# jhidalgocarrio/slam-localization

Hardware: AMD Instinct MI355X
Metric: filter predict+update steps/sec (higher is better)
Workload: dtype f64

## Files before the change

### slam-localization_amd/csrc/slk_step_fast.hpp

```cpp
#pragma once
#ifdef SLK_STAMPS
#define SLK_FSTAMP(i) do { SLK_STAMP_NR(i); if (a.stop > 0 && a.stop == (i)) return true; } while (0)
#define SLK_WSTAMP(w, i) do { if (tid == 64 * (w) && a.dbg) a.dbg[(size_t)bidx * 32 + (i)] = clock64(); } while (0)
#define SLK_FBAIL(code) do { SLK_NOTE(28, code); return false; } while (0)
#else
#define SLK_FSTAMP(i) do { } while (0)
#define SLK_WSTAMP(w, i) do { } while (0)
#define SLK_FBAIL(code) return false
#endif

namespace slk {

template <int K> struct FastShape {
    static constexpr int N = 12 + 6 * K, Nq = 13 + 7 * K, S = 2 * N + 1, NSO3 = K + 1;
    static constexpr int NT = (N + 15) / 16, NTL = NT * (NT + 1) / 2, NKS = (N + 3) / 4;
    static constexpr int NROT = 3 * NSO3;
    static constexpr int NP = 3 * K * K + 15 * K + 6;
    static constexpr int NIT = NP + NSO3;
    static constexpr int RND = (NIT + 255) / 256;
    static constexpr int oLt = 0;
    static constexpr int oMu = oLt + NTL * 256;
    static constexpr int oRef = oMu + ((Nq + 7) & ~7);
    static constexpr int oDelta = oRef + ((Nq + 7) & ~7);
    static constexpr int oMd = oDelta + 64;
    static constexpr int oD0 = oMd + 32;
    static constexpr int oD0s = oD0 + 32;
    static constexpr int oPd = oD0s + 32;
    static constexpr int oCq = oPd + 64;
    static constexpr int oStr = oCq + 40;
    static constexpr int oInts = oStr + 64;
    static constexpr int oTab = oInts + 32;
    static constexpr int oMsq = oTab + 28;
    static constexpr int oU = oTab + 32;
    static constexpr int uYp = 0, uW = 0, uDZ = 1088, uSm = 1600, uMdiag = 1664, uB = 1728, uInnov = 1792, uDz0 = 1800, uTmp = 1808;
    static constexpr int USZ = (NKS * 128 > 1936) ? NKS * 128 : 1936;
    static constexpr int total = oU + USZ;
};

static_assert(FastShape<8>::total * 8 * 4 <= 160 * 1024 && FastShape<7>::total * 8 * 4 <= 160 * 1024, "four workgroups per CU");

__host__ __device__ inline int fast_step_lds_doubles(int k)
{
    switch (k) {
    case 4: return FastShape<4>::total;
    case 5: return FastShape<5>::total;
    case 6: return FastShape<6>::total;
    case 7: return FastShape<7>::total;
    case 8: return FastShape<8>::total;
    default: return 0;
    }
}

__device__ __forceinline__ double wave_sum_f64(double x) { return readlane_f64(wave_inclusive_scan(x), 63); }

template <int N> __device__ __forceinline__ int fast_rho(int t)
{
    if (t >= N) return 31;
    if (t < 12) return (t >= 3 && t < 6) ? t - 3 : 31;
    const int cc = (t - 12) / 6, r = (t - 12) - 6 * cc;
    return r >= 3 ? 3 * cc + r : 31;
}
__device__ __forceinline__ int fast_vec_storage(int t)
{
    if (t < 12) return t < 3 ? t : (t < 6 ? -1 : t + 1);
    const int cc = (t - 12) / 6, r = (t - 12) - 6 * cc;
    return r < 3 ? 13 + 7 * cc + r : -1;
}

__device__ const double fast_series_table[26] = {
    0x1.1d8d32755f8fbp-29, 0x1.27e40964b47d4p-22, 0x1.a01a00fb1bc6fp-16, 0x1.6c16c16bdd04ep-10, 0x1.5555555555421p-5, 0x1.fffffffffffffp-2,
    0x1.ac53ce336f805p-26, 0x1.71dd113fb7905p-19, 0x1.a01a01061c190p-13, 0x1.11111110ecfb3p-7, 0x1.555555555548fp-3,
    0x1.78be0a9b1dd1fp-5, 0x1.0b3340fe2ed9ap-4, 0x1.3ab708d770276p-4, 0x1.7459b99bfc19bp-4, 0x1.c71c5f4b9c2adp-4, 0x1.24924907fa636p-3, 0x1.999999996d307p-3, 0x1.5555555555481p-2,
    0.0, 0.0, 0.0, 0.0, 0.0, 0.0, 0.0};

__device__ __forceinline__ bool wave_all(bool p) { return __builtin_amdgcn_ballot_w64(!p) == 0ull; }

template <int NV, bool WIDE>
__device__ __forceinline__ void so3_exp_tab_path(const double *T, const double (&v)[NV][3], const double (&x)[NV], Quat (&q)[NV])
{
    double y[NV], cc[NV], ss[NV];
#pragma unroll
    for (int i = 0; i < NV; ++i) y[i] = WIDE ? -0.0625 * x[i] : -x[i];
    {
        const double c0 = T[0], s0 = T[6];
#pragma unroll
        for (int i = 0; i < NV; ++i) { cc[i] = c0; ss[i] = s0; }
    }
#pragma unroll
    for (int k = 1; k < 5; ++k) {
        const double ck = T[k], sk = T[6 + k];
#pragma unroll
        for (int i = 0; i < NV; ++i) { cc[i] = fma(cc[i], y[i], ck); ss[i] = fma(ss[i], y[i], sk); }
    }
    {
        const double c5 = T[5];
#pragma unroll
        for (int i = 0; i < NV; ++i) {
            cc[i] = fma(cc[i], y[i], c5);
            cc[i] = fma(cc[i], y[i], 1.0);
            ss[i] = fma(ss[i], y[i], 1.0);
        }
    }
#pragma unroll
    for (int i = 0; i < NV; ++i) {
        double m = 0.5 * ss[i], w = cc[i];
        if (WIDE) {
            m *= 0.25;
#pragma unroll
            for (int rep = 0; rep < 2; ++rep) {
                const double w2 = fma(2.0 * w, w, -1.0);
                m = 2.0 * w * m;
                w = w2;
            }
        }
        q[i] = Quat{m * v[i][0], m * v[i][1], m * v[i][2], w};
    }
}
template <int NV, bool FLAG>
__device__ __forceinline__ bool so3_exp_tab_impl(const double *T, const double (&v)[NV][3], Quat (&q)[NV], int *flag)
{
    double x[NV];
    unsigned hm = 0;
#pragma unroll
    for (int i = 0; i < NV; ++i) {
        x[i] = 0.25 * (v[i][0] * v[i][0] + v[i][1] * v[i][1] + v[i][2] * v[i][2]);
        const unsigned hi = (unsigned)__double2hiint(x[i]);
        hm = hi > hm ? hi : hm;
    }
    if (wave_all(nonneg_hi_below(hm, HI_QUARTER))) {
        so3_exp_tab_path<NV, false>(T, v, x, q);
        return true;
    }
    so3_exp_tab_path<NV, true>(T, v, x, q);
    const bool ok = nonneg_hi_below(hm, HI_FOUR);
    if (!FLAG) return ok;
    if (!wave_all(ok)) *flag = 1;
    return true;
}
__device__ __forceinline__ Quat qmul_exp(const Quat &a, const Quat &b)
{
    Quat o;
    o.w = fma(-a.z, b.z, fma(-a.y, b.y, fma(a.w, b.w, -(a.x * b.x))));
    o.x = fma(-a.z, b.y, fma(a.y, b.z, fma(a.x, b.w, a.w * b.x)));
    o.y = fma(-a.x, b.z, fma(a.z, b.x, fma(a.y, b.w, a.w * b.y)));
    o.z = fma(-a.y, b.x, fma(a.x, b.y, fma(a.z, b.w, a.w * b.z)));
    return o;
}
template <int NV>
__device__ __forceinline__ bool so3_exp_tab(const double *T, const double (&v)[NV][3], Quat (&q)[NV])
{
    return so3_exp_tab_impl<NV, false>(T, v, q, nullptr);
}
template <int NV>
__device__ __forceinline__ void so3_exp_tab_flag(const double *T, const double (&v)[NV][3], Quat (&q)[NV], int *flag)
{
    so3_exp_tab_impl<NV, true>(T, v, q, flag);
}
template <int NV>
__device__ __forceinline__ bool so3_log_tab(const double *T, const Quat (&q)[NV], double (&d)[NV][3])
{
    double y[NV], sc[NV], f[NV];
    bool small = true;
#pragma unroll
    for (int i = 0; i < NV; ++i) {
        const double n2 = q[i].x * q[i].x + q[i].y * q[i].y + q[i].z * q[i].z, ws = q[i].w * fabs(q[i].w);
        small = small && (n2 * 16.0 < ws);
        y[i] = n2;
    }
    const bool wide = !wave_all(small);
    if (!wide) {
#pragma unroll
        for (int i = 0; i < NV; ++i) {
            const double r = rcp_refined(q[i].w);
            sc[i] = 2.0 * r;
            y[i] = -(y[i] * r * r);
        }
    } else {
#pragma unroll
        for (int i = 0; i < NV; ++i) {
            const double n2 = y[i], aw = fabs(q[i].w);
            const double r = rcp_refined(1.0 + aw);
            double k = r, t2 = n2 * r * r;
#pragma unroll
            for (int rep = 0; rep < 2; ++rep) {
                const double a1 = 1.0 + t2;
                double sq, rs;
                rsqrt_pivot(a1, sq, rs);
                const double den = fma(a1, rs, 1.0);
                const double rd = rcp_refined(den);
                k *= rd;
                t2 *= rd * rd;
            }
            sc[i] = (q[i].w < 0.0) ? -16.0 * k : 16.0 * k;
            y[i] = -t2;
        }
    }
    {
        const double a0 = T[11];
#pragma unroll
        for (int i = 0; i < NV; ++i) f[i] = a0;
    }
#pragma unroll
    for (int k = 1; k < 8; ++k) {
        const double ak = T[11 + k];
#pragma unroll
        for (int i = 0; i < NV; ++i) f[i] = fma(f[i], y[i], ak);
    }
#pragma unroll
    for (int i = 0; i < NV; ++i) {
        f[i] = fma(f[i], y[i], 1.0);
        const double sv = sc[i] * f[i];
        d[i][0] = sv * q[i].x; d[i][1] = sv * q[i].y; d[i][2] = sv * q[i].z;
    }
    return true;
}

template <int E0, int CNT>
__device__ __forceinline__ void fast_scan_entries(const double (&av)[8], double (&G)[20])
{
#pragma unroll
    for (int e = 0; e < CNT; ++e) {
        constexpr int dummy = 0; (void)dummy;
        const int q = E0 + e;
        const int r = (q >= 1) + (q >= 3) + (q >= 6) + (q >= 10) + (q >= 15) + (q >= 21) + (q >= 28), cc = q - r * (r + 1) / 2;
        const double pr = av[r] * av[cc];
        G[e] = wave_inclusive_scan(pr) - pr;
    }
}

template <int K> struct FastPairTable {
    unsigned long long v[FastShape<K>::NP];
    constexpr FastPairTable() : v{}
    {
        int p = 0;
        for (int b = 0; b <= K; ++b) {
            const int to = b ? 9 + 6 * b : 3;
            for (int j = 0; j < to + 3; ++j, ++p) {
                unsigned long long a[3] = {0, 0, 0};
                for (int cc = 0; cc < 3; ++cc) {
                    const int t = to + cc, I = t >> 4, Jc = j >> 4;
                    a[cc] = (unsigned long long)(FastShape<K>::oLt + (Jc <= I ? (I * (I + 1) / 2 + Jc) * 256 + (j & 15) * 16 + (t & 15) : 16));
                }
                const int rho = 3 * b;
                const unsigned long long e0 = (unsigned long long)(((j >> 2) * 2 + (rho >> 4)) * 64 + (j & 3) * 16 + (rho & 15));
                const unsigned long long sd = (b == 1 && j >= 16) ? (unsigned long long)(j - 15) : 0ull;
                v[p] = a[0] | (a[1] << 13) | ((unsigned long long)b << 26) | (sd << 30) | (a[2] << 32) | (e0 << 45);
            }
        }
    }
};
template <int K> struct FastPairTableHolder { static __device__ const FastPairTable<K> tab; };
template <int K> __device__ const FastPairTable<K> FastPairTableHolder<K>::tab = FastPairTable<K>();

#define SLK_G(r, c) Gf[(r) * ((r) + 1) / 2 + (c)]
__device__ __forceinline__ bool fast_ldm_columns(double (&Gf)[36], const double *dZi, const double *Sm, unsigned kept, int lane, int N,
                                                 double *Wb, double *mdiag)
{
    const bool live = lane < N;
    const bool full = kept == 0xffu;
    double y[8];
    bool ok = true;
#pragma unroll
    for (int j = 0; j < 8; ++j) {
        if (full) {
#pragma unroll
            for (int r = j; r < 8; ++r) SLK_G(r, j) = Sm[r + 8 * j] - SLK_G(r, j);
        } else {
            const bool kj = (kept >> j) & 1u;
#pragma unroll
            for (int r = j; r < 8; ++r) {
                const bool in = kj && ((kept >> r) & 1u);
                const double sv = Sm[in ? r + 8 * j : 0];
                SLK_G(r, j) = in ? sv - SLK_G(r, j) : ((r == j) ? 1.0 : 0.0);
            }
        }
        double d = SLK_G(j, j);
#pragma unroll
        for (int p = 0; p < j; ++p) d = fma(-SLK_G(j, p), SLK_G(j, p), d);
        ok = ok && (d > 0.0);
        double sq, rs;
        rsqrt_pivot(d, sq, rs);
        SLK_G(j, j) = rs;
#pragma unroll
        for (int i = j + 1; i < 8; ++i) {
            double v = SLK_G(i, j);
#pragma unroll
            for (int p = 0; p < j; ++p) v = fma(-SLK_G(i, p), SLK_G(j, p), v);
            SLK_G(i, j) = v * rs;
        }
        const double aj = dZi[(j >> 1) * 128 + 2 * lane + (j & 1)];
        double sacc = ((kept >> j) & 1u) ? 0.5 * aj : 0.0;
#pragma unroll
        for (int p = 0; p < j; ++p) sacc = fma(-SLK_G(j, p), y[p], sacc);
        y[j] = sacc * rs;
    }
    double dj = 1.0;
#pragma unroll
    for (int c = 0; c < 8; ++c) dj = fma(-y[c], y[c], dj);
    ok = ok && (dj > 0.0);
    double sqd, rsd;
    rsqrt_pivot(dj, sqd, rsd);
    const double sc = -0.5 * rsd;
#pragma unroll
    for (int c = 7; c >= 0; --c) {
        double sacc = y[c];
#pragma unroll
        for (int p = c + 1; p < 8; ++p) sacc = fma(-SLK_G(p, c), y[p], sacc);
        y[c] = sacc * SLK_G(c, c);
        Wb[bw_idx(lane, c)] = live ? y[c] * sc : 0.0;
    }
    mdiag[lane] = live ? sqd : 1.0;
    return __all(ok) != 0;
}
#undef SLK_G

template <int NT, class FillFn>
__device__ __forceinline__ void ldm_product_tiled(double *Lt, const double *dZi, const double *Wb, const double *mdiag, int lane,
                                                  int wave, int JB, FillFn fill)
{
    const int c = lane & 15, g = lane >> 4;
    const int lw = (g >> 1) * 128 + 2 * c + (g & 1);
    constexpr int MAXT = (NT == 4) ? 4 : 2;
    d4 acc[MAXT];
#pragma unroll
    for (int q = 0; q < MAXT; ++q) acc[q] = d4{0.0, 0.0, 0.0, 0.0};
#pragma unroll
    for (int I = 0; I < NT; ++I)
#pragma unroll
        for (int J = 0; J <= I; ++J) {
            if (ldm_tile_wave<NT>(I, J) != wave || J > JB) continue;
            d4 a = {0.0, 0.0, 0.0, 0.0};
            const double wf0 = Wb[32 * J + lw], wf1 = Wb[256 + 32 * J + lw];
#pragma unroll
            for (int Kb = J; Kb <= I; ++Kb) {
                if (Kb > JB) continue;
                d4 mt = {0.0, 0.0, 0.0, 0.0};
                const double a0 = dZi[32 * Kb + lw], a1 = dZi[256 + 32 * Kb + lw];
                double lf[4];
#pragma unroll
                for (int s = 0; s < 4; ++s) lf[s] = Lt[(I * (I + 1) / 2 + Kb) * 256 + 64 * s + lane];
                mt = __builtin_amdgcn_mfma_f64_16x16x4f64(a0, wf0, mt, 0, 0, 0);
                mt = __builtin_amdgcn_mfma_f64_16x16x4f64(a1, wf1, mt, 0, 0, 0);
                if (Kb == J) {
                    const double dg = mdiag[16 * J + c];
#pragma unroll
                    for (int r = 0; r < 4; ++r) {
                        const int row = g + 4 * r;
                        mt[r] = (row > c) ? mt[r] : ((row == c) ? dg : 0.0);
                    }
                }
#pragma unroll
                for (int s = 0; s < 4; ++s) a = __builtin_amdgcn_mfma_f64_16x16x4f64(mt[s], lf[s], a, 0, 0, 0);
            }
            acc[ldm_tile_slot<NT>(I, J)] = a;
        }
    __syncthreads();
#pragma unroll
    for (int I = 0; I < NT; ++I)
#pragma unroll
        for (int J = 0; J <= I; ++J) {
            if (ldm_tile_wave<NT>(I, J) != wave || J > JB) continue;
            const d4 a = acc[ldm_tile_slot<NT>(I, J)];
#pragma unroll
            for (int r = 0; r < 4; ++r) Lt[(I * (I + 1) / 2 + J) * 256 + 64 * r + lane] = a[r];
        }
    fill();
    __syncthreads();
}

template <int K> struct FastEE {
    using F = FastShape<K>;
    static constexpr int EES = 40;
    static constexpr int NTE = F::NROT > 16 ? 2 : 1;
    static constexpr int PAD = 16 * NTE - 1;
    static constexpr int BLO = F::NSO3 - 1 < 5 ? F::NSO3 - 1 : 5;
    static constexpr int CLO = (BLO ? 9 + 6 * BLO : 3) + 3;
    static constexpr int KS0 = ((CLO + 3) / 4 < F::NKS) ? (CLO + 3) / 4 : F::NKS;
    static constexpr int KS1 = F::NKS;
    __host__ __device__ static constexpr int wave_of(int hi, int hj) { return hi == 0 ? 0 : (hj == 0 ? 2 : 3); }
};
static_assert(32 * FastEE<8>::EES <= FastShape<4>::USZ, "EE fits the union region");

template <int K, int HI, int HJ>
__device__ __forceinline__ d4 fast_ee_tile(const double *Et, int lane)
{
    constexpr int KE = HJ == 0 ? FastEE<K>::KS0 : FastEE<K>::KS1;
    d4 acc = {0.0, 0.0, 0.0, 0.0};
#pragma unroll
    for (int ks = 0; ks < KE; ++ks) {
        const double fj = Et[ks * 128 + HJ * 64 + lane];
        const double fi = HI == HJ ? fj : Et[ks * 128 + HI * 64 + lane];
        acc = __builtin_amdgcn_mfma_f64_16x16x4f64(fi, fj, acc, 0, 0, 0);
    }
    return acc;
}
template <int K, int HI, int HJ>
__device__ __forceinline__ void fast_ee_publish(double *ee, int lane, const d4 &acc)
{
    constexpr int EES = FastEE<K>::EES;
    const int c = lane & 15, g = lane >> 4;
#pragma unroll
    for (int r = 0; r < 4; ++r) {
        ee[(16 * HI + g + 4 * r) * EES + 16 * HJ + c] = acc[r];
        if (HI != HJ) ee[(16 * HJ + c) * EES + 16 * HI + g + 4 * r] = acc[r];
    }
}

template <int K> __host__ __device__ constexpr unsigned fast_rho_pack(int I, int G)
{
    constexpr int N = FastShape<K>::N, PAD = FastEE<K>::PAD;
    unsigned w = 0;
    for (int r = 0; r < 4; ++r) {
        const int t = 16 * I + G + 4 * r;
        int rho = PAD;
        if (t < N) {
            if (t < 12) rho = (t >= 3 && t < 6) ? t - 3 : PAD;
            else { const int cc = (t - 12) / 6, q = (t - 12) - 6 * cc; rho = q >= 3 ? 3 * cc + q : PAD; }
        }
        w |= (unsigned)rho << (8 * r);
    }
    return w;
}

template <int K, int J>
__device__ __forceinline__ void fast_rebuild_col(const double *Lt, const double *str, int lane, d4 (&acc)[FastShape<K>::NT])
{
    using F = FastShape<K>;
    constexpr int NT = F::NT;
    constexpr int KEND = (4 * J + 4 + (J == 0 ? 1 : 0) < F::NKS) ? 4 * J + 4 + (J == 0 ? 1 : 0) : F::NKS;
#pragma unroll
    for (int ks = 0; ks < KEND; ++ks) {
        double fo[NT];
#pragma unroll
        for (int I = J; I < NT; ++I) {
            const int Kc = ks >> 2;
            fo[I] = (Kc <= I) ? Lt[(I * (I + 1) / 2 + Kc) * 256 + (ks & 3) * 64 + lane] : str[lane];
        }
#pragma unroll
        for (int I = J; I < NT; ++I) acc[I - J] = __builtin_amdgcn_mfma_f64_16x16x4f64(fo[I], fo[J], acc[I - J], 0, 0, 0);
    }
}

template <int K, int J>
__device__ __forceinline__ void fast_store_col(const double *pd, const double *ee, double *bufs, double *oP, int lane,
                                               d4 (&acc)[FastShape<K>::NT], bool lower_only)
{
    using F = FastShape<K>;
    constexpr int NT = F::NT, N = F::N, EES = FastEE<K>::EES, PAD = FastEE<K>::PAD;
    const int c = lane & 15, g = lane >> 4;
    {
        const int rj = fast_rho<N>(16 * J + c);
        const double bf = pd[g == 0 ? 32 + rj : (g == 1 ? rj : 31)];
#pragma unroll
        for (int I = J; I < NT; ++I) {
            const int ri = fast_rho<N>(16 * I + c);
            const double af = pd[g == 0 ? ri : (g == 1 ? 32 + ri : 31)];
            acc[I - J] = __builtin_amdgcn_mfma_f64_16x16x4f64(af, bf, acc[I - J], 0, 0, 0);
        }
        const double *eec = ee + (rj & PAD);
#pragma unroll
        for (int I = J; I < NT; ++I) {
            const unsigned rw = g == 0 ? fast_rho_pack<K>(I, 0) : (g == 1 ? fast_rho_pack<K>(I, 1) : (g == 2 ? fast_rho_pack<K>(I, 2) : fast_rho_pack<K>(I, 3)));
#pragma unroll
            for (int r = 0; r < 4; ++r) acc[I - J][r] += eec[((rw >> (8 * r)) & 0xffu) * EES];
        }
    }
    double *o = oP + c + g * N;
#pragma unroll
    for (int I = J; I < NT; ++I) {
#pragma unroll
        for (int r = 0; r < 4; ++r) {
            const bool full = 16 * I + 4 * r + 3 < N && 16 * J + 15 < N;
            if (I > J && lower_only) continue;
            if (16 * I + 4 * r < N && (full || (16 * I + 4 * r + g < N && 16 * J + c < N)))
                o[16 * J + (16 * I + 4 * r) * N] = acc[I - J][r];
        }
        if (I > J) {
            double *buf = bufs + (I * (I - 1) / 2 + J) * 272;
#pragma unroll
            for (int r = 0; r < 4; ++r) buf[c * 17 + g + 4 * r] = acc[I - J][r];
            wave_sync();
#pragma unroll
            for (int q = 0; q < 4; ++q) {
                const double v = buf[(g + 4 * q) * 17 + c];
                const bool full = 16 * I + 15 < N;
                if (full || 16 * I + c < N) o[16 * I + (16 * J + 4 * q) * N] = v;
            }
        }
    }
}

template <int K>
__device__ __forceinline__ bool msckf_step_fast(const KArgs &a, double *smem)
{
    using F = FastShape<K>;
    constexpr int N = F::N, Nq = F::Nq, S = F::S, NSO3 = F::NSO3, NT = F::NT, NKS = F::NKS, NROT = F::NROT;
    constexpr int NP = F::NP;
    constexpr int NTHREADS = 256;
    if (a.mm != SLK_MM_FEATURE_PROJ || a.gate == 2 || a.emit != 0 || a.rebuild_prec != 0 || !a.mp || a.m != 8) return false;
    const int bidx = blockIdx.x, tid = threadIdx.x, lane = tid & 63;
    const int wave = __builtin_amdgcn_readfirstlane(tid >> 6);
    const int c16 = lane & 15, g4 = lane >> 4;
    double *Lt = smem + F::oLt, *mu = smem + F::oMu, *ref = smem + F::oRef, *delta = smem + F::oDelta, *md32 = smem + F::oMd;
    double *d0 = smem + F::oD0, *d0s = smem + F::oD0s, *pd = smem + F::oPd, *cq = smem + F::oCq, *str = smem + F::oStr, *U = smem + F::oU;
    int *ints = reinterpret_cast<int *>(smem + F::oInts);
    double *T = smem + F::oTab, *msq = smem + F::oMsq;
    double *Yp = U + F::uYp, *Wb = U + F::uW, *dZi = U + F::uDZ, *Sm = U + F::uSm, *mdiag = U + F::uMdiag, *bvec = U + F::uB;
    double *innov = U + F::uInnov, *dz0 = U + F::uDz0, *tmpS = U + F::uTmp, *Et = U;
    const double *gmean = a.mean + (size_t)bidx * Nq;
    const double *gP = a.P + (size_t)bidx * N * N;
    const double *mp = a.mp + (size_t)bidx * a.mp_stride;
    SLK_STAMP_NR(0);

    int jmax = 0, bad;
    const bool here = a.wsfail == nullptr;
    {
        const double *gL = here ? gP : a.wsL + (size_t)bidx * pk_size(N);
        const int t = lane, It = t >> 4;
        const int lbase = (It * (It + 1) / 2) * 256 + wave * 16 + (t & 15);
        double v[16];
        if (!here) {
#pragma unroll
            for (int u = 0; u < 16; ++u) {
                const int j = 4 * u + wave;
                const bool in = j < N && t >= j && t < N;
                v[u] = gL[in ? pkcol(N, j) + t : 0];
            }
        }
        const double mu0 = (tid < Nq) ? gmean[tid] : 0.0;
        const int t0 = (tid && tid < NSO3) ? 9 + 6 * tid : 3;
        const double pdg = gP[t0 * (N + 1)] + gP[(t0 + 1) * (N + 1)] + gP[(t0 + 2) * (N + 1)];
        const double tabv = fast_series_table[tid < 26 ? tid : 25];
        bad = here ? 0 : (a.wsfail[bidx] >= 0);
        bool ok = true;
#pragma unroll
        for (int f = 0; f < 4; ++f) {
            const double cf = mp[4 * f + 3];
            ok = ok && (cf >= 0.0) && (cf <= (double)K);
            const int cp = ok ? (int)cf : 0, tp = cp ? 6 + 6 * cp : 0;
            jmax = (tp + 5 > jmax) ? tp + 5 : jmax;
        }
        bad |= !ok;
        if (tid < NSO3) bad |= !(pdg < 9.869604401089358);
        if (tid < Nq) mu[tid] = mu0;
        if (tid < 64) { str[tid] = 0.0; pd[tid] = 0.0; ints[tid] = 0; }
        if (tid < 32) { d0[tid] = 0.0; md32[tid] = 0.0; }
        if (tid < 26) T[tid] = tabv;
        if (!here) {
#pragma unroll
            for (int u = 0; u < 16; ++u) {
                const int j = 4 * u + wave;
                const bool in = j < N && t >= j && t < N;
                if ((u >> 2) < NT && It >= (u >> 2) && It < NT) Lt[lbase + (u >> 2) * 256 + (u & 3) * 64] = in ? v[u] : 0.0;
            }
        }
        if (here) {
            d4 fa[CholM<NT>::NTL];
            if (wave == 0) cholm_load_t_exact<NT, N>(fa, gP, lane);
            else {
                double2 *Lt2 = reinterpret_cast<double2 *>(Lt);
                for (int e = tid - 64; e < CholM<NT>::NTL * 128; e += NTHREADS - 64) Lt2[e] = double2{0.0, 0.0};
            }
            __syncthreads();
            if (wave == 0) bad |= cholp_factor<NT, 2, N>(fa, Lt, N, U, lane) >= 0;
        }
    }
    if (__syncthreads_or(bad)) SLK_FBAIL(2);
    SLK_FSTAMP(3);

    {
        const int f = wave;
        const int cp = (int)mp[4 * f + 3];
        const int tp = cp ? 6 + 6 * cp : 0, sp = cp ? 6 + 7 * cp : 0;
        const double fx = mp[4 * f], fy = mp[4 * f + 1], fz = mp[4 * f + 2];
        const int j = lane, Jc = j >> 4;
        const bool act = j < tp + 6;
        double l[6], x[7];
#pragma unroll
        for (int q = 0; q < 6; ++q) {
            const int t = tp + q, I = t >> 4;
            const bool in = act && Jc <= I;
            l[q] = Lt[in ? (I * (I + 1) / 2 + Jc) * 256 + (j & 15) * 16 + (t & 15) : 16];
        }
#pragma unroll
        for (int q = 0; q < 7; ++q) x[q] = mu[sp + q];
        double zp0, zp1, zm0, zm1;
        {
            const double rv[2][3] = {{l[3], l[4], l[5]}, {-l[3], -l[4], -l[5]}};
            Quat ex[2];
            so3_exp_tab_flag<2>(T, rv, ex, ints + 50);
            const Quat qx = Quat{x[3], x[4], x[5], x[6]};
            double lx, ly, lz;
            auto quot = [](double lx_, double ly_, double lz_, double &q0, double &q1) __attribute__((always_inline)) {
                const double r = rcp_refined(lz_);
                q0 = lx_ * r; q0 = fma(fma(-lz_, q0, lx_), r, q0);
                q1 = ly_ * r; q1 = fma(fma(-lz_, q1, ly_), r, q1);
            };
            qrot(qconj(qmul_exp(qx, ex[0])), fx - (x[0] + l[0]), fy - (x[1] + l[1]), fz - (x[2] + l[2]), lx, ly, lz);
            quot(lx, ly, lz, zp0, zp1);
            qrot(qconj(qmul_exp(qx, ex[1])), fx - (x[0] - l[0]), fy - (x[1] - l[1]), fz - (x[2] - l[2]), lx, ly, lz);
            quot(lx, ly, lz, zm0, zm1);
        }
        const double Z00 = readlane_f64(zp0, 63), Z01 = readlane_f64(zp1, 63);
        const double yp0 = zp0 - Z00, yp1 = zp1 - Z01, ym0 = zm0 - Z00, ym1 = zm1 - Z01;
        Yp[j * 17 + 2 * f] = yp0; Yp[j * 17 + 2 * f + 1] = yp1;
        Yp[j * 17 + 8 + 2 * f] = ym0; Yp[j * 17 + 8 + 2 * f + 1] = ym1;
        dZi[f * 128 + 2 * j] = yp0 - ym0; dZi[f * 128 + 2 * j + 1] = yp1 - ym1;
        const double s0 = wave_sum_f64(yp0 + ym0), s1 = wave_sum_f64(yp1 + ym1);
        if (lane == 0) {
            const double e0 = s0 * (1.0 / (double)S), e1 = s1 * (1.0 / (double)S);
            innov[2 * f] = a.z[(size_t)bidx * 8 + 2 * f] - (Z00 + e0);
            innov[2 * f + 1] = a.z[(size_t)bidx * 8 + 2 * f + 1] - (Z01 + e1);
            dz0[2 * f] = e0; dz0[2 * f + 1] = e1;
        }
    }
    __syncthreads();
    if (ints[50]) SLK_FBAIL(3);
    SLK_FSTAMP(4);

    double Gs[20];
    if (wave == 1) {
        d4 acc = {0.0, 0.0, 0.0, 0.0};
#pragma unroll
        for (int ks = 0; ks < NKS; ++ks) {
            const double fr = Yp[ks * 68 + g4 * 17 + c16];
            acc = __builtin_amdgcn_mfma_f64_16x16x4f64(fr, fr, acc, 0, 0, 0);
        }
        if (c16 < 8) { tmpS[g4 + 8 * c16] = acc[0]; tmpS[g4 + 4 + 8 * c16] = acc[1]; }
        else { tmpS[64 + g4 + 8 * (c16 - 8)] = acc[2]; tmpS[64 + g4 + 4 + 8 * (c16 - 8)] = acc[3]; }
        wave_sync();
        const double *R = a.R + (size_t)bidx * a.r_stride;
        const int row = lane & 7, col = lane >> 3;
        Sm[lane] = 0.5 * ((tmpS[lane] + tmpS[64 + lane]) - (double)S * dz0[row] * dz0[col]) + R[lane];
    } else if (wave >= 2) {
        double av[8];
#pragma unroll
        for (int cc = 0; cc < 8; ++cc) av[cc] = 0.5 * dZi[(cc >> 1) * 128 + 2 * lane + (cc & 1)];
        if (wave == 2) fast_scan_entries<0, 16>(av, Gs);
        else fast_scan_entries<16, 20>(av, Gs);
        SLK_WSTAMP(3, 21);
    }
    __syncthreads();
    SLK_FSTAMP(6);

    unsigned kept = 0xffu, nout = 0u;
    if (a.gate) {
        const int p = 2 * (lane & 3), q = p + 1;
        const double s00 = Sm[p + 8 * p], s01 = Sm[p + 8 * q], s10 = Sm[q + 8 * p], s11 = Sm[q + 8 * q];
        const double det = s00 * s11 - s01 * s10, r0 = innov[p], r1 = innov[q];
        const double d2 = (r0 * (s11 * r0 - s01 * r1) + r1 * (s00 * r1 - s10 * r0)) / det;
        if (!__all(d2 < 5.99)) {
            int *ix = ints + 10 * wave;
            if (lane == 0) {
                int cnt = 8, i = 0;
                unsigned no = 0;
                for (int r = 0; r < 8; ++r) ix[r] = r;
                while (i < cnt / 2) {
                    const int pp = ix[2 * i], qq = ix[2 * i + 1];
                    const double t00 = Sm[pp + 8 * pp], t01 = Sm[pp + 8 * qq], t10 = Sm[qq + 8 * pp], t11 = Sm[qq + 8 * qq];
                    const double dt = t00 * t11 - t01 * t10, u0 = innov[pp], u1 = innov[qq];
                    const double dd = (u0 * (t11 * u0 - t01 * u1) + u1 * (t00 * u1 - t10 * u0)) / dt;
                    if (!(dd < 5.99)) {
                        for (int rep = 0; rep < 2; ++rep) {
                            const int pos = 2 * i + rep, numRows = cnt - 1;
                            if (pos < numRows) for (int w = pos; w < numRows; ++w) ix[w] = ix[w + 1];
                            cnt = numRows;
                        }
                        no++;
                    } else {
                        i++;
                    }
                }
                unsigned kp = 0;
                for (int r = 0; r < cnt; ++r) kp |= 1u << ix[r];
                ix[8] = (int)kp; ix[9] = (int)no;
            }
            wave_sync();
            kept = (unsigned)ix[8]; nout = (unsigned)ix[9];
        }
    }
    if (kept == 0u) SLK_FBAIL(4);
    SLK_FSTAMP(7);

    if (wave == 2) {
#pragma unroll
        for (int e = 0; e < 16; ++e) Yp[e * 64 + lane] = Gs[e];
    }
    __syncthreads();
    if (wave == 0) {
        double gg[8][8], gi[8], y[8];
        if (kept == 0xffu) {
#pragma unroll
            for (int i = 0; i < 8; ++i) {
#pragma unroll
                for (int j = 0; j <= i; ++j) gg[i][j] = Sm[i + 8 * j];
            }
        } else {
#pragma unroll
            for (int i = 0; i < 8; ++i) {
#pragma unroll
                for (int j = 0; j <= i; ++j) {
                    const bool in = ((kept >> i) & 1u) && ((kept >> j) & 1u);
                    const double v = Sm[in ? i + 8 * j : 0];
                    gg[i][j] = in ? v : (i == j ? 1.0 : 0.0);
                }
            }
        }
        bool spd = true;
#pragma unroll
        for (int j = 0; j < 8; ++j) {
            double d = gg[j][j];
#pragma unroll
            for (int p = 0; p < j; ++p) d = fma(-gg[j][p], gg[j][p], d);
            spd = spd && (d > 0.0);
            double sq, rs;
            rsqrt_pivot(d, sq, rs);
            gi[j] = rs;
#pragma unroll
            for (int i = j + 1; i < 8; ++i) {
                double v = gg[i][j];
#pragma unroll
                for (int p = 0; p < j; ++p) v = fma(-gg[i][p], gg[j][p], v);
                gg[i][j] = v * rs;
            }
            double s = ((kept >> j) & 1u) ? innov[j] : 0.0;
#pragma unroll
            for (int p = 0; p < j; ++p) s = fma(-gg[j][p], y[p], s);
            y[j] = s * rs;
        }
#pragma unroll
        for (int cc = 7; cc >= 0; --cc) {
            double s = y[cc];
#pragma unroll
            for (int p = cc + 1; p < 8; ++p) s = fma(-gg[p][cc], y[p], s);
            y[cc] = s * gi[cc];
        }
        if (!spd && lane == 0) ints[49] = 1;
        SLK_WSTAMP(0, 24);
        double bj = 0.0;
#pragma unroll
        for (int cc = 0; cc < 8; ++cc) bj = fma(dZi[(cc >> 1) * 128 + 2 * lane + (cc & 1)], y[cc], bj);
        bvec[lane] = 0.5 * bj;
        wave_sync();
        {
            const int t = lane, It = t >> 4;
            const double *Lrow = Lt + (It * (It + 1) / 2) * 256 + (t & 15);
            double part[NT];
#pragma unroll
            for (int Jb = 0; Jb < NT; ++Jb) {
                double s = 0.0;
#pragma unroll
                for (int jj = 0; jj < 16; ++jj) {
                    if (16 * Jb + jj < N) s = fma(Lrow[Jb * 256 + jj * 16], bvec[16 * Jb + jj], s);
                    if ((jj & 7) == 7) __builtin_amdgcn_sched_barrier(0);
                }
                part[Jb] = s;
            }
            double dl = part[0];
#pragma unroll
            for (int Jb = 1; Jb < NT; ++Jb) dl += (It >= Jb) ? part[Jb] : 0.0;
            if (t < 64) delta[t] = (t < N) ? dl : 0.0;
            const int s = (t < N) ? fast_vec_storage(t) : -1;
            if (s >= 0) ref[s] = mu[s] + dl;
        }
        wave_sync();
        if (lane < NSO3) {
            const int to = lane ? 9 + 6 * lane : 3, so = lane ? 9 + 7 * lane : 3;
            const Quat qm = ldq(mu + so);
            const double dv[1][3] = {{delta[to], delta[to + 1], delta[to + 2]}};
            Quat ex[1];
            so3_exp_tab_flag<1>(T, dv, ex, ints + 50);
            const Quat qr = qmul_exp(qm, ex[0]);
            stq(ref + so, qr);
            stq(cq + 4 * lane, qmul(qconj(qr), qm));
        }
        SLK_WSTAMP(0, 25);
    }
    else if (wave == 3) {
        SLK_WSTAMP(3, 22);
        double Gf[36];
#pragma unroll
        for (int e = 0; e < 16; ++e) Gf[e] = Yp[e * 64 + lane];
#pragma unroll
        for (int e = 16; e < 36; ++e) Gf[e] = Gs[e - 16];
        const bool pdok = fast_ldm_columns(Gf, dZi, Sm, kept, lane, N, Wb, mdiag);
        if (!pdok && lane == 0) ints[48] = 1;
        SLK_WSTAMP(3, 23);
    }
    __syncthreads();
    if (ints[48] | ints[49] | ints[50]) SLK_FBAIL(5);
    SLK_FSTAMP(8);

    unsigned long long pt0 = 0, pt1 = 0;
    ldm_product_tiled<NT>(Lt, dZi, Wb, mdiag, lane, wave, jmax >> 4, [&]() {
        pt0 = FastPairTableHolder<K>::tab.v[tid < NP ? tid : 0];
        pt1 = FastPairTableHolder<K>::tab.v[(wave == 1 && 256 + lane < NP) ? 256 + lane : 0];
        for (int e = tid; e < NKS * 128; e += 256) Et[e] = 0.0;
    });
    SLK_FSTAMP(11);

    constexpr int RP = (NP + 255) / 256;
    int aL[RP][3], aE0[RP], bsd[RP];
    bool val[RP];
#pragma unroll
    for (int r = 0; r < RP; ++r) {
        const unsigned long long w = r ? pt1 : pt0;
        const unsigned lo = (unsigned)w, hi = (unsigned)(w >> 32);
        val[r] = (r ? 256 + lane : tid) < NP && (r == 0 || wave == 1);
        bsd[r] = lo >> 26;
        aL[r][0] = lo & 0x1fff; aL[r][1] = (lo >> 13) & 0x1fff; aL[r][2] = hi & 0x1fff;
        aE0[r] = (hi >> 13) & 0x7ff;
    }
    auto e_off = [](int e0, int b, int cc) __attribute__((always_inline)) {
        const int rho = 3 * b;
        const int e1 = e0 + ((rho & 15) == 15 ? 49 : 1);
        return cc == 0 ? e0 : (cc == 1 ? e1 : e1 + (((rho + 1) & 15) == 15 ? 49 : 1));
    };
    double dpl[RP][3], dmi[RP][3], dc[3] = {0.0, 0.0, 0.0};
    int it = 0;
    for (;;) {
#pragma unroll
        for (int r = 0; r < RP; ++r) {
            if (r == 0 ? 64 * wave >= NP : wave != 1) continue;
            const int b = bsd[r] & 15, to = b ? 9 + 6 * b : 3;
            const double l0 = smem[aL[r][0]], l1 = smem[aL[r][1]], l2 = smem[aL[r][2]];
            const double e0 = delta[to], e1 = delta[to + 1], e2 = delta[to + 2];
            const Quat cb = ldq(cq + 4 * b);
            const double rv[2][3] = {{e0 + l0, e1 + l1, e2 + l2}, {e0 - l0, e1 - l1, e2 - l2}};
            Quat ex[2];
            double dd[2][3];
            so3_exp_tab_flag<2>(T, rv, ex, ints + 50);
            ex[0] = qmul_exp(cb, ex[0]);
            ex[1] = qmul_exp(cb, ex[1]);
#ifdef SLK_STAMPS
            {
                bool se = true, sl = true;
                for (int i = 0; i < 2; ++i) {
                    se = se && (0.25 * (rv[i][0] * rv[i][0] + rv[i][1] * rv[i][1] + rv[i][2] * rv[i][2]) < 0.25);
                    const double n2 = ex[i].x * ex[i].x + ex[i].y * ex[i].y + ex[i].z * ex[i].z;
                    sl = sl && (ex[i].w > 0.0) && (n2 * 16.0 < ex[i].w * ex[i].w);
                }
                const int code = (__all(se) ? 0 : 1) | (__all(sl) ? 0 : 2);
                const int slot = wave < 2 ? 26 + wave : 27 + wave;
                if (lane == 0 && a.dbg && it == 0) a.dbg[(size_t)bidx * 32 + slot] = (r ? a.dbg[(size_t)bidx * 32 + slot] : 0) | (code << (2 * r));
            }
#endif
            so3_log_tab<2>(T, ex, dd);
#pragma unroll
            for (int cc = 0; cc < 3; ++cc) { dpl[r][cc] = dd[0][cc]; dmi[r][cc] = dd[1][cc]; }
            if (val[r]) {
#pragma unroll
                for (int cc = 0; cc < 3; ++cc) Et[e_off(aE0[r], b, cc)] = 0.5 * (dpl[r][cc] + dmi[r][cc]);
            }
        }
        if (wave == 2) {
            const int b = lane < NSO3 ? lane : 0, to = b ? 9 + 6 * b : 3;
            const double rv[1][3] = {{delta[to], delta[to + 1], delta[to + 2]}};
            const Quat cb = ldq(cq + 4 * b);
            Quat ex[1];
            double dd[1][3];
            so3_exp_tab_flag<1>(T, rv, ex, ints + 50);
            ex[0] = qmul_exp(cb, ex[0]);
            so3_log_tab<1>(T, ex, dd);
#pragma unroll
            for (int cc = 0; cc < 3; ++cc) {
                dc[cc] = dd[0][cc];
                if (lane < NSO3) {
                    d0[3 * b + cc] = dc[cc];
                    d0s[3 * b + cc] = (double)(S - 2 * (b ? 12 + 6 * b : 6)) * dc[cc];
                }
            }
        }
        __syncthreads();
        if (ints[50]) SLK_FBAIL(6);
        if (wave >= 2) {
            const int hr = wave - 2;
            double s = 0.0;
#pragma unroll
            for (int ks = 0; ks < NKS; ++ks) s += Et[(ks * 2 + hr) * 64 + lane];
            s += __shfl_xor(s, 16, 64);
            s += __shfl_xor(s, 32, 64);
            const int rho = 16 * hr + lane;
            double sq = 0.0;
            if (lane < 16 && rho < NROT) {
                const double mv = (2.0 * s + d0s[rho]) * (1.0 / (double)S);
                md32[rho] = mv;
                sq = mv * mv;
            }
            sq += dpp_mov_f64<0x111, 0xf>(sq);
            sq += dpp_mov_f64<0x112, 0xf>(sq);
            sq += dpp_mov_f64<0x114, 0xf>(sq);
            sq += dpp_mov_f64<0x118, 0xf>(sq);
            if (lane == 15) msq[hr] = sq;
        }
        __syncthreads();
        const bool more = __builtin_amdgcn_ballot_w64(msq[0] + msq[1] > MEAN_STOP_SQ) != 0ull;
        if (wave == 0 && lane < NSO3) {
            const int so = lane ? 9 + 7 * lane : 3;
            const double dv[1][3] = {{md32[3 * lane], md32[3 * lane + 1], md32[3 * lane + 2]}};
            Quat ex[1];
            so3_exp_tab_flag<1>(T, dv, ex, ints + 50);
            const Quat qr = qmul_exp(ldq(ref + so), ex[0]);
            stq(ref + so, qr);
            stq(cq + 4 * lane, qmul(qconj(qr), ldq(mu + so)));
        }
        if (!more) break;
        if (++it >= 64) SLK_FBAIL(7);
        __syncthreads();
    }
    SLK_FSTAMP(12);
    SLK_NOTE(20, it + 1);
    {
        auto fix = [&](double &x, double &y, double &z, double m0, double m1, double m2) __attribute__((always_inline)) {
            const double cx = y * m2 - z * m1, cy = z * m0 - x * m2, cz = x * m1 - y * m0;
            const double ax = y * cz - z * cy, ay = z * cx - x * cz, az = x * cy - y * cx;
            const double a12 = 1.0 / 12.0 + (x * x + y * y + z * z) * (1.0 / 720.0);
            x = x - m0 + 0.5 * cx - a12 * ax;
            y = y - m1 + 0.5 * cy - a12 * ay;
            z = z - m2 + 0.5 * cz - a12 * az;
        };
#pragma unroll
        for (int r = 0; r < RP; ++r) {
            if (r == 0 ? 64 * wave >= NP : wave != 1) continue;
            const int b = bsd[r] & 15, sd = bsd[r] >> 4;
            const double m0 = md32[3 * b], m1 = md32[3 * b + 1], m2 = md32[3 * b + 2];
            double c0 = d0[3 * b], c1 = d0[3 * b + 1], c2 = d0[3 * b + 2];
            fix(c0, c1, c2, m0, m1, m2);
            fix(dpl[r][0], dpl[r][1], dpl[r][2], m0, m1, m2);
            fix(dmi[r][0], dmi[r][1], dmi[r][2], m0, m1, m2);
            if (val[r]) {
                smem[sd ? F::oStr + 16 * sd - 1 : aL[r][0]] = 0.5 * (dpl[r][0] - dmi[r][0]);
                smem[aL[r][1]] = 0.5 * (dpl[r][1] - dmi[r][1]);
                smem[aL[r][2]] = 0.5 * (dpl[r][2] - dmi[r][2]);
                Et[e_off(aE0[r], b, 0)] = 0.5 * (dpl[r][0] + dmi[r][0]) - c0;
                Et[e_off(aE0[r], b, 1)] = 0.5 * (dpl[r][1] + dmi[r][1]) - c1;
                Et[e_off(aE0[r], b, 2)] = 0.5 * (dpl[r][2] + dmi[r][2]) - c2;
            }
        }
        if (wave == 2 && lane < NSO3) {
            fix(dc[0], dc[1], dc[2], md32[3 * lane], md32[3 * lane + 1], md32[3 * lane + 2]);
            pd[32 + 3 * lane] = dc[0]; pd[32 + 3 * lane + 1] = dc[1]; pd[32 + 3 * lane + 2] = dc[2];
        }
    }
    __syncthreads();
    if (ints[50]) SLK_FBAIL(8);
    double *omean = a.mean_out ? a.mean_out + (size_t)bidx * Nq : a.mean + (size_t)bidx * Nq;
    double *oP = a.P_out ? a.P_out + (size_t)bidx * N * N : a.P + (size_t)bidx * N * N;
    if (wave == 1 && lane < N) {
        const int sv = fast_vec_storage(lane);
        if (sv >= 0) omean[sv] = ref[sv];
    }
    if (wave == 0 && lane < NSO3) {
        const int so = lane ? 9 + 7 * lane : 3;
        const Quat qr = ldq(ref + so);
        omean[so] = qr.x; omean[so + 1] = qr.y; omean[so + 2] = qr.z; omean[so + 3] = qr.w;
    }
    if (tid == 0) a.outliers[bidx] = nout;
    SLK_FSTAMP(13);

    if (wave >= 2) {
        const int hr = wave - 2;
        double s = 0.0;
#pragma unroll
        for (int ks = 0; ks < NKS; ++ks) s += Et[(ks * 2 + hr) * 64 + lane];
        s += __shfl_xor(s, 16, 64);
        s += __shfl_xor(s, 32, 64);
        const int rho = 16 * hr + lane;
        if (lane < 16 && rho < NROT) pd[rho] = s + (0.5 * ((double)N + 0.5)) * pd[32 + rho];
    }
    using EE = FastEE<K>;
    static_assert(NROT <= EE::PAD && EE::wave_of(0, 0) == 0 && EE::wave_of(1, 0) == 2 && EE::wave_of(1, 1) == 3, "EE tiles");
    d4 eacc = {0.0, 0.0, 0.0, 0.0};
    if (wave == 0) eacc = fast_ee_tile<K, 0, 0>(Et, lane);
    else if constexpr (EE::NTE > 1) {
        if (wave == 2) eacc = fast_ee_tile<K, 1, 0>(Et, lane);
        else if (wave == 3) eacc = fast_ee_tile<K, 1, 1>(Et, lane);
    }
    __syncthreads();
    double *ee = U;
    if (wave == 0) fast_ee_publish<K, 0, 0>(ee, lane, eacc);
    else if constexpr (EE::NTE > 1) {
        if (wave == 2) fast_ee_publish<K, 1, 0>(ee, lane, eacc);
        else if (wave == 3) fast_ee_publish<K, 1, 1>(ee, lane, eacc);
    }
    d4 acc[NT];
#pragma unroll
    for (int q = 0; q < NT; ++q) acc[q] = d4{0.0, 0.0, 0.0, 0.0};
    if (wave == 0) fast_rebuild_col<K, 0>(Lt, str, lane, acc);
    else if (wave == 1) fast_rebuild_col<K, 1>(Lt, str, lane, acc);
    else if (wave == 2) fast_rebuild_col<K, 2>(Lt, str, lane, acc);
    else if constexpr (NT > 3) fast_rebuild_col<K, 3>(Lt, str, lane, acc);
    __syncthreads();
    SLK_FSTAMP(14);
    if (wave == 0) fast_store_col<K, 0>(pd, ee, Lt, oP, lane, acc, a.lower_only != 0);
    else if (wave == 1) fast_store_col<K, 1>(pd, ee, Lt, oP, lane, acc, a.lower_only != 0);
    else if (wave == 2) fast_store_col<K, 2>(pd, ee, Lt, oP, lane, acc, a.lower_only != 0);
    else if constexpr (NT > 3) fast_store_col<K, 3>(pd, ee, Lt, oP, lane, acc, a.lower_only != 0);
    SLK_STAMP_NR(15);
    return true;
}

}
```

Baseline: 24.96 million.

## Reassign LDM tiles per wave sharing column products, fold rank-2 update into EE tiles

The blocked L·D·M product is restructured so each wave owns tiles grouped by column J. It computes the dZi·W product for each (J,Kb) block once and reuses it across every output row tile I it owns, instead of recomputing it per tile. The tile-to-wave mapping changes and the accumulator count drops for NT=4. Separately, the rank-2 rotation correction is applied once to the small EE tiles before they are published, rather than per output tile in the store phase. This cuts redundant MFMAs but may shift load balance between waves.

Measured after the change: 25.30 million, median of 6. +1.3%, better.

```diff
diff --git a/slam-localization_amd/csrc/slk_step_fast.hpp b/slam-localization_amd/csrc/slk_step_fast.hpp
--- a/slam-localization_amd/csrc/slk_step_fast.hpp
+++ b/slam-localization_amd/csrc/slk_step_fast.hpp
@@ -314,53 +314,86 @@
 }
 #undef SLK_G
 
+template <int NT> __host__ __device__ constexpr int fast_ldm_wave(int I, int J)
+{
+    if (NT == 4) return J == 0 ? ((I == 3 || I == 0) ? 0 : 1) : (J == 1 ? 2 : 3);
+    return J == 0 ? (I == 2 ? 2 : 0) : (J == 1 ? 1 : 3);
+}
+template <int NT> __host__ __device__ constexpr int fast_ldm_slot(int I, int J)
+{
+    int n = 0;
+    for (int i = 0; i < NT; ++i)
+        for (int j = 0; j <= i; ++j) {
+            if (i == I && j == J) return n;
+            if (fast_ldm_wave<NT>(i, j) == fast_ldm_wave<NT>(I, J)) ++n;
+        }
+    return n;
+}
+template <int NT> __host__ __device__ constexpr bool fast_ldm_owns(int W, int J, int K0)
+{
+    for (int i = (K0 > J ? K0 : J); i < NT; ++i)
+        if (fast_ldm_wave<NT>(i, J) == W) return true;
+    return false;
+}
+
+template <int NT, int W, int MAXT>
+__device__ __forceinline__ void fast_ldm_wave_tiles(const double *Lt, const double *dZi, const double *Wb, const double *mdiag, int lane,
+                                                    int JB, d4 (&acc)[MAXT])
+{
+    const int c = lane & 15, g = lane >> 4;
+    const int lw = (g >> 1) * 128 + 2 * c + (g & 1);
+#pragma unroll
+    for (int J = 0; J < NT; ++J) {
+        if (!fast_ldm_owns<NT>(W, J, J) || J > JB) continue;
+        const double wf0 = Wb[32 * J + lw], wf1 = Wb[256 + 32 * J + lw];
+#pragma unroll
+        for (int Kb = J; Kb < NT; ++Kb) {
+            if (!fast_ldm_owns<NT>(W, J, Kb) || Kb > JB) continue;
+            d4 mt = {0.0, 0.0, 0.0, 0.0};
+            const double a0 = dZi[32 * Kb + lw], a1 = dZi[256 + 32 * Kb + lw];
+            mt = __builtin_amdgcn_mfma_f64_16x16x4f64(a0, wf0, mt, 0, 0, 0);
+            mt = __builtin_amdgcn_mfma_f64_16x16x4f64(a1, wf1, mt, 0, 0, 0);
+            if (Kb == J) {
+                const double dg = mdiag[16 * J + c];
+#pragma unroll
+                for (int r = 0; r < 4; ++r) {
+                    const int row = g + 4 * r;
+                    mt[r] = (row > c) ? mt[r] : ((row == c) ? dg : 0.0);
+                }
+            }
+#pragma unroll
+            for (int I = Kb; I < NT; ++I) {
+                if (fast_ldm_wave<NT>(I, J) != W) continue;
+                double lf[4];
+#pragma unroll
+                for (int s = 0; s < 4; ++s) lf[s] = Lt[(I * (I + 1) / 2 + Kb) * 256 + 64 * s + lane];
+                d4 &a = acc[fast_ldm_slot<NT>(I, J)];
+#pragma unroll
+                for (int s = 0; s < 4; ++s) a = __builtin_amdgcn_mfma_f64_16x16x4f64(mt[s], lf[s], a, 0, 0, 0);
+            }
+        }
+    }
+}
+
 template <int NT, class FillFn>
 __device__ __forceinline__ void ldm_product_tiled(double *Lt, const double *dZi, const double *Wb, const double *mdiag, int lane,
                                                   int wave, int JB, FillFn fill)
 {
-    const int c = lane & 15, g = lane >> 4;
-    const int lw = (g >> 1) * 128 + 2 * c + (g & 1);
-    constexpr int MAXT = (NT == 4) ? 4 : 2;
+    constexpr int MAXT = (NT == 4) ? 3 : 2;
     d4 acc[MAXT];
 #pragma unroll
     for (int q = 0; q < MAXT; ++q) acc[q] = d4{0.0, 0.0, 0.0, 0.0};
+    if (wave == 0) fast_ldm_wave_tiles<NT, 0>(Lt, dZi, Wb, mdiag, lane, JB, acc);
+    else if (wave == 1) fast_ldm_wave_tiles<NT, 1>(Lt, dZi, Wb, mdiag, lane, JB, acc);
+    else if (wave == 2) fast_ldm_wave_tiles<NT, 2>(Lt, dZi, Wb, mdiag, lane, JB, acc);
+    else fast_ldm_wave_tiles<NT, 3>(Lt, dZi, Wb, mdiag, lane, JB, acc);
+    __syncthreads();
 #pragma unroll
     for (int I = 0; I < NT; ++I)
 #pragma unroll
         for (int J = 0; J <= I; ++J) {
-            if (ldm_tile_wave<NT>(I, J) != wave || J > JB) continue;
-            d4 a = {0.0, 0.0, 0.0, 0.0};
-            const double wf0 = Wb[32 * J + lw], wf1 = Wb[256 + 32 * J + lw];
-#pragma unroll
-            for (int Kb = J; Kb <= I; ++Kb) {
-                if (Kb > JB) continue;
-                d4 mt = {0.0, 0.0, 0.0, 0.0};
-                const double a0 = dZi[32 * Kb + lw], a1 = dZi[256 + 32 * Kb + lw];
-                double lf[4];
-#pragma unroll
-                for (int s = 0; s < 4; ++s) lf[s] = Lt[(I * (I + 1) / 2 + Kb) * 256 + 64 * s + lane];
-                mt = __builtin_amdgcn_mfma_f64_16x16x4f64(a0, wf0, mt, 0, 0, 0);
-                mt = __builtin_amdgcn_mfma_f64_16x16x4f64(a1, wf1, mt, 0, 0, 0);
-                if (Kb == J) {
-                    const double dg = mdiag[16 * J + c];
-#pragma unroll
-                    for (int r = 0; r < 4; ++r) {
-                        const int row = g + 4 * r;
-                        mt[r] = (row > c) ? mt[r] : ((row == c) ? dg : 0.0);
-                    }
-                }
-#pragma unroll
-                for (int s = 0; s < 4; ++s) a = __builtin_amdgcn_mfma_f64_16x16x4f64(mt[s], lf[s], a, 0, 0, 0);
-            }
-            acc[ldm_tile_slot<NT>(I, J)] = a;
-        }
-    __syncthreads();
-#pragma unroll
-    for (int I = 0; I < NT; ++I)
-#pragma unroll
-        for (int J = 0; J <= I; ++J) {
-            if (ldm_tile_wave<NT>(I, J) != wave || J > JB) continue;
-            const d4 a = acc[ldm_tile_slot<NT>(I, J)];
+            if (fast_ldm_wave<NT>(I, J) != wave || J > JB) continue;
+            const d4 a = acc[fast_ldm_slot<NT>(I, J)];
 #pragma unroll
             for (int r = 0; r < 4; ++r) Lt[(I * (I + 1) / 2 + J) * 256 + 64 * r + lane] = a[r];
         }
@@ -394,6 +427,14 @@
     }
     return acc;
 }
+template <int HI, int HJ>
+__device__ __forceinline__ d4 fast_ee_rank2(const double *pd, int lane, const d4 &acc)
+{
+    const int c = lane & 15, g = lane >> 4;
+    const double af = pd[g == 0 ? 16 * HI + c : (g == 1 ? 32 + 16 * HI + c : 31)];
+    const double bf = pd[g == 0 ? 32 + 16 * HJ + c : (g == 1 ? 16 * HJ + c : 31)];
+    return __builtin_amdgcn_mfma_f64_16x16x4f64(af, bf, acc, 0, 0, 0);
+}
 template <int K, int HI, int HJ>
 __device__ __forceinline__ void fast_ee_publish(double *ee, int lane, const d4 &acc)
 {
@@ -442,21 +483,14 @@
 }
 
 template <int K, int J>
-__device__ __forceinline__ void fast_store_col(const double *pd, const double *ee, double *bufs, double *oP, int lane,
-                                               d4 (&acc)[FastShape<K>::NT], bool lower_only)
+__device__ __forceinline__ void fast_store_col(const double *ee, double *bufs, double *oP, int lane, d4 (&acc)[FastShape<K>::NT],
+                                               bool lower_only)
 {
     using F = FastShape<K>;
     constexpr int NT = F::NT, N = F::N, EES = FastEE<K>::EES, PAD = FastEE<K>::PAD;
     const int c = lane & 15, g = lane >> 4;
     {
         const int rj = fast_rho<N>(16 * J + c);
-        const double bf = pd[g == 0 ? 32 + rj : (g == 1 ? rj : 31)];
-#pragma unroll
-        for (int I = J; I < NT; ++I) {
-            const int ri = fast_rho<N>(16 * I + c);
-            const double af = pd[g == 0 ? ri : (g == 1 ? 32 + ri : 31)];
-            acc[I - J] = __builtin_amdgcn_mfma_f64_16x16x4f64(af, bf, acc[I - J], 0, 0, 0);
-        }
         const double *eec = ee + (rj & PAD);
 #pragma unroll
         for (int I = J; I < NT; ++I) {
@@ -978,10 +1012,10 @@
     }
     __syncthreads();
     double *ee = U;
-    if (wave == 0) fast_ee_publish<K, 0, 0>(ee, lane, eacc);
+    if (wave == 0) fast_ee_publish<K, 0, 0>(ee, lane, fast_ee_rank2<0, 0>(pd, lane, eacc));
     else if constexpr (EE::NTE > 1) {
-        if (wave == 2) fast_ee_publish<K, 1, 0>(ee, lane, eacc);
-        else if (wave == 3) fast_ee_publish<K, 1, 1>(ee, lane, eacc);
+        if (wave == 2) fast_ee_publish<K, 1, 0>(ee, lane, fast_ee_rank2<1, 0>(pd, lane, eacc));
+        else if (wave == 3) fast_ee_publish<K, 1, 1>(ee, lane, fast_ee_rank2<1, 1>(pd, lane, eacc));
     }
     d4 acc[NT];
 #pragma unroll
@@ -992,10 +1026,10 @@
     else if constexpr (NT > 3) fast_rebuild_col<K, 3>(Lt, str, lane, acc);
     __syncthreads();
     SLK_FSTAMP(14);
-    if (wave == 0) fast_store_col<K, 0>(pd, ee, Lt, oP, lane, acc, a.lower_only != 0);
-    else if (wave == 1) fast_store_col<K, 1>(pd, ee, Lt, oP, lane, acc, a.lower_only != 0);
-    else if (wave == 2) fast_store_col<K, 2>(pd, ee, Lt, oP, lane, acc, a.lower_only != 0);
-    else if constexpr (NT > 3) fast_store_col<K, 3>(pd, ee, Lt, oP, lane, acc, a.lower_only != 0);
+    if (wave == 0) fast_store_col<K, 0>(ee, Lt, oP, lane, acc, a.lower_only != 0);
+    else if (wave == 1) fast_store_col<K, 1>(ee, Lt, oP, lane, acc, a.lower_only != 0);
+    else if (wave == 2) fast_store_col<K, 2>(ee, Lt, oP, lane, acc, a.lower_only != 0);
+    else if constexpr (NT > 3) fast_store_col<K, 3>(ee, Lt, oP, lane, acc, a.lower_only != 0);
     SLK_STAMP_NR(15);
     return true;
 }
```
